# enoche/MMRec

Hardware: AMD Instinct MI355X
Metric: GCN-layer edges/sec (3-layer user-item CSR SpMM, d=64, fp32) (higher is better)
Workload: dtype f32

## Files before the change

include/mmrec_hip.h:

```cpp
#ifndef MMREC_HIP_H
#define MMREC_HIP_H

#include <stddef.h>
#include <stdint.h>

#ifdef __cplusplus
extern "C" {
#endif

#define MMREC_ABI_VERSION 16
#define MMREC_EMB_DIM 64

#define MMREC_ERR_BAD_ARG 10001
#define MMREC_ERR_UNSUPPORTED 10002

typedef void* mmrec_stream_t;

int mmrec_abi_version(void);
const char* mmrec_error_string(int err);

#ifndef MMREC_SPMM_CHUNK
#define MMREC_SPMM_CHUNK 512
#endif
#define MMREC_SPMM_LONG_ROW_DEFAULT 32

int mmrec_spmm_csr_f32(const int32_t* rowptr, const int32_t* colidx, const float* vals,
                       const float* X, float* Y, const float* Z, const float* acc_in, float* acc_out,
                       int32_t n_rows, int32_t d, float alpha, float beta, float acc_scale,
                       int32_t long_row_threshold, const int32_t* long_rows,
                       const int32_t* long_chunk_ptr, int32_t n_long, int32_t n_chunks,
                       float* partials, int32_t* long_tickets, mmrec_stream_t stream);

int mmrec_spmm_rows_f32(const int32_t* rowptr, const int32_t* colidx, const float* vals, const float* X,
                        const float* Z, int32_t z_compact, const int64_t* rows, int32_t n_list, int32_t d,
                        int32_t long_row_threshold, float* Y, mmrec_stream_t stream);
int mmrec_spmm_rows_any_f32(const int32_t* rowptr, const int32_t* colidx, const float* vals, const float* X,
                            const float* Z, int32_t z_compact, const int64_t* rows, int32_t n_list, int32_t d,
                            int32_t long_row_threshold, int32_t max_row_chunks, float* Y, mmrec_stream_t stream);
int mmrec_spmm_push_rows_f32(const int32_t* rowptr, const int32_t* colidx, const float* vals, const float* G,
                             float g_scale, const int64_t* rows, int32_t n_list, int32_t d, float* dX, float* dZ,
                             mmrec_stream_t stream);

int mmrec_spmm_csr_f32_layergcn(const int32_t* rowptr, const int32_t* colidx, const float* vals, const float* X,
                                float* Y, const float* ego, float* scaled, float* w, const float* acc_in,
                                float* acc_out, int32_t n_rows, int32_t d, int32_t long_row_threshold,
                                const int32_t* long_rows, const int32_t* long_chunk_ptr, int32_t n_long,
                                int32_t n_chunks, float* partials, int32_t* long_tickets, mmrec_stream_t stream);
int mmrec_spmm_csr_sched_f32(const int32_t* rowptr, const int32_t* colidx, const float* vals, const float* X, float* Y,
                             const float* Z, const float* acc_in, float* acc_out, int32_t n_rows, int32_t d, float alpha,
                             float beta, float acc_scale, int32_t long_row_threshold, const int32_t* long_rows,
                             const int32_t* long_chunk_ptr, int32_t n_long, int32_t n_chunks, float* partials,
                             int32_t* long_tickets, const int32_t* sched_row, const int32_t* sched_span,
                             const int32_t* sched_col, const float* sched_val, int32_t n_short, mmrec_stream_t stream);
int mmrec_spmm_csr_sched_f32_layergcn(const int32_t* rowptr, const int32_t* colidx, const float* vals, const float* X,
                                      float* Y, const float* ego, float* scaled, float* w, const float* acc_in,
                                      float* acc_out, int32_t n_rows, int32_t d, int32_t long_row_threshold,
                                      const int32_t* long_rows, const int32_t* long_chunk_ptr, int32_t n_long,
                                      int32_t n_chunks, float* partials, int32_t* long_tickets, const int32_t* sched_row,
                                      const int32_t* sched_span, const int32_t* sched_col, const float* sched_val,
                                      int32_t n_short, mmrec_stream_t stream);
int mmrec_spmm_row_keys(const int32_t* rowptr, const int32_t* colidx, const int32_t* col_degree, int32_t n_rows,
                        int32_t long_row_threshold, int32_t key_deg_max, int32_t* key, int32_t* key_degree,
                        mmrec_stream_t stream);

int mmrec_spmm_csr_masked_f32(const int32_t* rowptr, const int32_t* colidx, const float* vals, const float* X, float* Y,
                              const float* Z, const float* acc_in, float* acc_out, int32_t n_rows, int32_t d, float alpha,
                              float beta, float acc_scale, int32_t long_row_threshold, const int32_t* long_rows,
                              const int32_t* long_chunk_ptr, int32_t n_long, int32_t n_chunks, float* partials,
                              int32_t* long_tickets, const uint32_t* keep_bits, float val_scale, mmrec_stream_t stream);
int mmrec_edge_keep_bits(const uint8_t* keep, int64_t n_edges, const int64_t* perm_a, uint32_t* bits_a,
                         const int64_t* perm_b, uint32_t* bits_b, mmrec_stream_t stream);
int mmrec_spmm_plan_count(const int32_t* rowptr_host, int32_t n_rows, int32_t long_row_threshold,
                          int32_t* n_long, int32_t* n_chunks);
int mmrec_spmm_plan_fill(const int32_t* rowptr_host, int32_t n_rows, int32_t long_row_threshold,
                         int32_t* long_rows, int32_t* long_chunk_ptr);

int mmrec_cos_scale_fwd_f32(const float* E, const float* Ego, float* Out, float* w, float* acc,
                            int32_t n_rows, int32_t d, mmrec_stream_t stream);
int mmrec_cos_scale_bwd_f32(const float* dOut, const float* E, const float* Ego, const float* w,
                            float* dE, float* dEgo_accum, int32_t n_rows, int32_t d,
                            mmrec_stream_t stream);

#define MMREC_BPR_LOGSIG 0
#define MMREC_BPR_GAMMA 1

size_t mmrec_bpr_workspace_bytes(int32_t batch);
int mmrec_bpr_fwd_f32(const float* U, const float* P, const float* N, const int64_t* users,
                      const int64_t* pos, const int64_t* neg, int32_t batch, int32_t d,
                      int32_t variant, float scale, float* loss_out, float* coef, void* workspace,
                      mmrec_stream_t stream);
int mmrec_bpr_bwd_f32(const float* U, const float* P, const float* N, const int64_t* users,
                      const int64_t* pos, const int64_t* neg, int32_t batch, int32_t d,
                      const float* coef, const float* grad_scalar, float scale, float* dU, float* dP,
                      float* dN, mmrec_stream_t stream);

int mmrec_bpr_dots_f32(const float* U, const float* P, const float* N, const int64_t* users,
                       const int64_t* pos, const int64_t* neg, int32_t batch, int32_t d, float* dots,
                       mmrec_stream_t stream);
int mmrec_bpr_loss_from_dots_f32(const float* dots, int32_t batch, int32_t variant, float scale,
                                 float* loss_out, float* coef, void* workspace, mmrec_stream_t stream);

int mmrec_gather_sqnorm_fwd_f32(const float* E, const int64_t* ids, int32_t batch, int32_t d,
                                float* out, void* workspace, mmrec_stream_t stream);
int mmrec_gather_scale_add_bwd_f32(const float* E, const int64_t* ids, int32_t batch, int32_t d,
                                   const float* coef_scalar, float* dE, mmrec_stream_t stream);
#define MMREC_ROWS_REG_MAX_TERMS 6
size_t mmrec_rows_reg_workspace_bytes(int32_t n_terms, int32_t max_batch);
int mmrec_rows_reg_fwd_f32(const float* const* E, const int64_t* const* ids, const int32_t* batch, int32_t n_terms, int32_t d,
                           int32_t mode, float scale, float* out, float* coef, void* workspace, mmrec_stream_t stream);
int mmrec_rows_reg_bwd_f32(const float* const* E, const int64_t* const* ids, const int32_t* batch, int32_t n_terms, int32_t d,
                           const float* coef, const float* g, float* const* dE, mmrec_stream_t stream);

#define MMREC_BPR_MAX_TERMS 4
size_t mmrec_bpr_multi_workspace_bytes(int32_t n_terms, int32_t batch);
int mmrec_bpr_multi_fwd_f32(const float* U, const int64_t* users, const float* const* I, const int64_t* const* pos,
                            const int64_t* const* neg, const float* w, int32_t n_terms, int32_t batch, int32_t d, int32_t variant,
                            float scale, float* total, float* losses, float* coef, void* workspace, mmrec_stream_t stream);
int mmrec_bpr_multi_bwd_f32(const float* U, const int64_t* users, const float* const* I, const int64_t* const* pos,
                            const int64_t* const* neg, const float* w, int32_t n_terms, int32_t batch, int32_t d, const float* coef,
                            const float* grad_scalar, float scale, float* dU, float* const* dI, mmrec_stream_t stream);

#define MMREC_COSINE_MAX_TERMS 8
size_t mmrec_cosine_multi_workspace_bytes(int32_t n_terms, int32_t max_batch);
int mmrec_cosine_multi_fwd_f32(const float* const* X, const int64_t* const* ix, const float* const* Y, const int64_t* const* iy,
                               const float* w, const int32_t* batch, int32_t n_terms, int32_t d, float* out, float* coef,
                               void* workspace, mmrec_stream_t stream);
int mmrec_cosine_multi_bwd_f32(const float* const* X, const int64_t* const* ix, const float* const* Y, const int64_t* const* iy,
                               const float* w, const int32_t* batch, int32_t n_terms, int32_t d, const float* coef,
// ... 229 lines not shown
```

mmrec_amd/_lib.py:

```python
from __future__ import annotations

import ctypes
import os
from ctypes import c_char_p, c_float, c_int32, c_int64, c_size_t, c_uint64, c_void_p

import torch

_PKG = os.path.dirname(os.path.abspath(__file__))
LIB_PATH = os.environ.get("MMREC_HIP_LIB") or os.path.join(_PKG, "lib", "libmmrec_hip.so")
ABI_VERSION = 16

_P = c_void_p

SIGNATURES = {
    "mmrec_abi_version": (c_int32, []),
    "mmrec_error_string": (c_char_p, [c_int32]),
    "mmrec_spmm_csr_f32": (c_int32, [_P, _P, _P, _P, _P, _P, _P, _P, c_int32, c_int32, c_float,
                                     c_float, c_float, c_int32, _P, _P, c_int32, c_int32, _P, _P, _P]),
    "mmrec_spmm_csr_f32_layergcn": (c_int32, [_P, _P, _P, _P, _P, _P, _P, _P, _P, _P, c_int32, c_int32, c_int32,
                                              _P, _P, c_int32, c_int32, _P, _P, _P]),
    "mmrec_spmm_csr_sched_f32": (c_int32, [_P, _P, _P, _P, _P, _P, _P, _P, c_int32, c_int32, c_float,
                                           c_float, c_float, c_int32, _P, _P, c_int32, c_int32, _P, _P,
                                           _P, _P, _P, _P, c_int32, _P]),
    "mmrec_spmm_csr_sched_f32_layergcn": (c_int32, [_P, _P, _P, _P, _P, _P, _P, _P, _P, _P, c_int32, c_int32, c_int32,
                                                    _P, _P, c_int32, c_int32, _P, _P, _P, _P, _P, _P, c_int32, _P]),
    "mmrec_spmm_csr_masked_f32": (c_int32, [_P, _P, _P, _P, _P, _P, _P, _P, c_int32, c_int32, c_float,
                                            c_float, c_float, c_int32, _P, _P, c_int32, c_int32, _P, _P, _P, c_float, _P]),
    "mmrec_edge_keep_bits": (c_int32, [_P, c_int64, _P, _P, _P, _P, _P]),
    "mmrec_spmm_row_keys": (c_int32, [_P, _P, _P, c_int32, c_int32, c_int32, _P, _P, _P]),
    "mmrec_spmm_plan_count": (c_int32, [_P, c_int32, c_int32, _P, _P]),
    "mmrec_spmm_plan_fill": (c_int32, [_P, c_int32, c_int32, _P, _P]),
    "mmrec_cos_scale_fwd_f32": (c_int32, [_P, _P, _P, _P, _P, c_int32, c_int32, _P]),
    "mmrec_cos_scale_bwd_f32": (c_int32, [_P, _P, _P, _P, _P, _P, c_int32, c_int32, _P]),
    "mmrec_bpr_workspace_bytes": (c_size_t, [c_int32]),
    "mmrec_bpr_fwd_f32": (c_int32, [_P, _P, _P, _P, _P, _P, c_int32, c_int32, c_int32, c_float, _P,
                                    _P, _P, _P]),
    "mmrec_spmm_rows_f32": (c_int32, [_P, _P, _P, _P, _P, c_int32, _P, c_int32, c_int32, c_int32, _P, _P]),
    "mmrec_spmm_rows_any_f32": (c_int32, [_P, _P, _P, _P, _P, c_int32, _P, c_int32, c_int32, c_int32, c_int32, _P, _P]),
    "mmrec_spmm_push_rows_f32": (c_int32, [_P, _P, _P, _P, c_float, _P, c_int32, c_int32, _P, _P, _P]),
    "mmrec_bpr_dots_f32": (c_int32, [_P, _P, _P, _P, _P, _P, c_int32, c_int32, _P, _P]),
    "mmrec_bpr_loss_from_dots_f32": (c_int32, [_P, c_int32, c_int32, c_float, _P, _P, _P, _P]),
    "mmrec_bpr_bwd_f32": (c_int32, [_P, _P, _P, _P, _P, _P, c_int32, c_int32, _P, _P, c_float, _P, _P,
                                    _P, _P]),
    "mmrec_gather_sqnorm_fwd_f32": (c_int32, [_P, _P, c_int32, c_int32, _P, _P, _P]),
    "mmrec_gather_scale_add_bwd_f32": (c_int32, [_P, _P, c_int32, c_int32, _P, _P, _P]),
    "mmrec_infonce_workspace_bytes": (c_size_t, [c_int32]),
    "mmrec_infonce_fwd_f32": (c_int32, [_P, _P, _P, c_int32, c_int32, c_float, _P, _P, _P]),
    "mmrec_infonce_bwd_f32": (c_int32, [_P, c_int32, c_int32, c_float, _P, _P, _P, _P, _P]),
    "mmrec_linear_workspace_bytes": (c_size_t, [c_int32, c_int32, c_int32]),
    "mmrec_linear_fwd_f32": (c_int32, [_P, _P, _P, _P, c_int32, c_int32, c_int32, _P, _P]),
    "mmrec_linear_fwd_split_f32": (c_int32, [_P, _P, _P, _P, c_int32, c_int32, c_int32, _P, _P]),
    "mmrec_linear_bwd_split_workspace_bytes": (c_size_t, [c_int32, c_int32, c_int32]),
    "mmrec_linear_bwd_split_f32": (c_int32, [_P, _P, _P, _P, _P, _P, c_int32, c_int32, c_int32, _P, _P]),
    "mmrec_linear_bwd_w_f32": (c_int32, [_P, _P, _P, _P, c_int32, c_int32, c_int32, _P, _P]),
    "mmrec_linear_bwd_x_f32": (c_int32, [_P, _P, _P, c_int32, c_int32, c_int32, _P]),
    "mmrec_linear_rows_workspace_bytes": (c_size_t, [c_int32, c_int32, c_int32]),
    "mmrec_linear_rows_fwd_f32": (c_int32, [_P, c_int64, _P, _P, _P, _P, c_int32, c_int32, c_int32, c_int32, _P, _P]),
    "mmrec_linear_rows_bwd_f32": (c_int32, [_P, _P, c_int64, _P, _P, _P, _P, _P, c_int32, c_int32, c_int32, _P, _P]),
    "mmrec_edge_dot_f32": (c_int32, [_P, c_int64, _P, c_int64, _P, _P, c_int64, c_int32, _P, _P]),
    "mmrec_edge_dot_bwd_f32": (c_int32, [_P, _P, c_int64, _P, c_int64, _P, _P, c_int64, c_int32, _P, _P, _P]),
    "mmrec_segment_softmax_group_max": (c_int32, []),
    "mmrec_segment_softmax_f32": (c_int32, [_P, c_int32, _P, _P, c_int32, _P, c_int64, c_float, _P, _P]),
    "mmrec_segment_softmax_bwd_f32": (c_int32, [_P, c_int32, _P, _P, c_int32, _P, _P, c_int64, _P, _P]),
    "mmrec_edge_attention_group_max": (c_int32, []),
    "mmrec_edge_attention_f32": (c_int32, [_P, c_int32, _P, _P, _P, c_int32, _P, c_int64, _P, c_int64, c_int32, c_int64, c_float,
                                           _P, _P, _P]),
    "mmrec_edge_attention_bwd_f32": (c_int32, [_P, c_int32, _P, _P, _P, c_int32, _P, _P, _P, _P, c_int32, _P, c_int64, _P, c_int64,
                                               _P, _P, _P, _P, c_int32, c_int64, _P, _P, _P, _P, _P]),
    "mmrec_neighbor_max_group_max": (c_int32, []),
    "mmrec_neighbor_max_f32": (c_int32, [_P, c_int32, _P, _P, _P, c_int32, _P, c_int64, c_int32, c_int64, _P, _P, _P]),
    "mmrec_neighbor_max_bwd_f32": (c_int32, [_P, c_int32, _P, _P, _P, c_int32, _P, c_int64, _P, c_int32, c_int64, _P, _P, _P]),
    "mmrec_score_lse_split_cols": (c_int32, [c_int32, c_int32, c_int32]),
    "mmrec_score_lse_workspace_bytes": (c_size_t, [c_int32, c_int32, c_int32]),
    "mmrec_score_lse_f32": (c_int32, [_P, _P, c_int32, c_int32, c_int32, c_float, _P, _P, _P]),
    "mmrec_score_lse_bwd_f32": (c_int32, [_P, _P, c_int32, c_int32, c_int32, c_float, _P, _P, _P, _P, _P, _P]),
    "mmrec_hyper_rows_per_block": (c_int32, [c_int64]),
    "mmrec_hyper_workspace_bytes": (c_size_t, [c_int64, c_int64, c_int32]),
    "mmrec_hyper_assign_fwd_f32": (c_int32, [_P, _P, _P, c_int64, c_int32, c_float, c_float, _P, _P, _P]),
    "mmrec_hyper_assign_bwd_f32": (c_int32, [_P, _P, _P, c_int64, c_int32, c_float, c_float, _P, _P]),
    "mmrec_hyper_layer_fwd_f32": (c_int32, [_P, _P, _P, c_int64, c_int64, c_int32, c_int32, _P, _P, _P, _P, _P]),
    "mmrec_hyper_layer_bwd_f32": (c_int32, [_P, _P, _P, _P, _P, _P, c_int64, c_int64, c_int32, c_int32, _P, _P, _P, _P, _P]),
    "mmrec_spectrum_rows_per_block": (c_int32, [c_int64]),
    "mmrec_spectrum_workspace_bytes": (c_size_t, [c_int64]),
    "mmrec_spectrum_fwd_f32": (c_int32, [_P, _P, _P, _P, _P, c_int64, c_int32, _P, _P, _P, _P]),
# ... 102 lines not shown
```

mmrec_amd/csrc/spmm.hip:

```cpp
#include "common.h"
#include "spmm_narrow.h"

#ifndef MMREC_SPMM_RPG
#define MMREC_SPMM_RPG(n_rows) ((n_rows) <= (1 << 18) ? 1 : 4)
#endif

namespace {

__device__ __forceinline__ void st_coherent(float4* p, float4 v) {
    unsigned long long* q = reinterpret_cast<unsigned long long*>(p);
    const unsigned long long lo = ((unsigned long long)__float_as_uint(v.y) << 32) | __float_as_uint(v.x);
    const unsigned long long hi = ((unsigned long long)__float_as_uint(v.w) << 32) | __float_as_uint(v.z);
    __hip_atomic_store(q, lo, __ATOMIC_RELAXED, __HIP_MEMORY_SCOPE_AGENT);
    __hip_atomic_store(q + 1, hi, __ATOMIC_RELAXED, __HIP_MEMORY_SCOPE_AGENT);
}
__device__ __forceinline__ float4 ld_coherent(const float4* p) {
    unsigned long long* q = reinterpret_cast<unsigned long long*>(const_cast<float4*>(p));
    const unsigned long long lo = __hip_atomic_load(q, __ATOMIC_RELAXED, __HIP_MEMORY_SCOPE_AGENT);
    const unsigned long long hi = __hip_atomic_load(q + 1, __ATOMIC_RELAXED, __HIP_MEMORY_SCOPE_AGENT);
    return make_float4(__uint_as_float((unsigned)lo), __uint_as_float((unsigned)(lo >> 32)),
                       __uint_as_float((unsigned)hi), __uint_as_float((unsigned)(hi >> 32)));
}

struct RowEpilogue {
// ... 151 lines not shown
            } else {
#pragma unroll
                for (int ch = 0; ch < DCH; ++ch) {
                    float4* dst = reinterpret_cast<float4*>(partials) + (size_t)chunk * (16 * DCH) + ch * 16 + lane16;
                    if (tickets) st_coherent(dst, t[ch]); else *dst = t[ch];
                }
            }
        }
        const int c0 = long_chunk_ptr[lo], c1 = long_chunk_ptr[lo + 1];
        if (!tickets || c1 - c0 == 1) return;
        if (threadIdx.x < 64) {
            __atomic_signal_fence(__ATOMIC_SEQ_CST);
            __builtin_amdgcn_s_waitcnt(0);
            __atomic_signal_fence(__ATOMIC_SEQ_CST);
            __builtin_amdgcn_fence(__ATOMIC_RELEASE, "workgroup");
            if (threadIdx.x == 0)
                s_last = __hip_atomic_fetch_add(tickets + lo, 1, __ATOMIC_RELAXED, __HIP_MEMORY_SCOPE_AGENT) == c1 - c0 - 1;
        }
        __syncthreads();
        if (!s_last) return;
        __builtin_amdgcn_fence(__ATOMIC_ACQUIRE, "workgroup");
        reduce_long_row<DCH, true, LG>(partials, c0, c1, row, ep, red);
        if (threadIdx.x == 0) __hip_atomic_store(tickets + lo, 0, __ATOMIC_RELAXED, __HIP_MEMORY_SCOPE_AGENT);
        return;
    }
    if (SCHED) {
        const int slot0 = ((int)blockIdx.x - n_chunks) * 16 * rows_per_group + g;
#pragma unroll 1
        for (int i = 0; i < rows_per_group; ++i) {
            const int slot = slot0 + i * 16;
            if (slot >= sched.n_short) break;
            const int row = sched.row[slot];
            const int2 se = sched.span[slot];
            float4 acc[DCH];
#pragma unroll
            for (int ch = 0; ch < DCH; ++ch) acc[ch] = f4_zero();
            gather_span<DCH>(sched.col, sched.val, X4, se.x, se.y, lane16, acc);
            store_row<DCH, LG>(ep, row, lane16, acc);
        }
        return;
    }
    const int row0 = ((int)blockIdx.x - n_chunks) * 16 * rows_per_group + g;
#pragma unroll 1
    for (int i = 0; i < rows_per_group; ++i) {
        const int row = row0 + i * 16;
        if (row >= n_rows) break;
        const int s = rowptr[row], e = rowptr[row + 1];
        if (e - s > long_t) continue;
        float4 acc[DCH];
#pragma unroll
        for (int ch = 0; ch < DCH; ++ch) acc[ch] = f4_zero();
        gather_span<DCH>(colidx, vals, X4, s, e, lane16, acc);
        store_row<DCH, LG>(ep, row, lane16, acc);
    }
}

template <int DCH, bool LG>
__global__ __launch_bounds__(256) void spmm_long_reduce_kernel(
    const int32_t* __restrict__ long_rows, const int32_t* __restrict__ long_chunk_ptr, int n_long,
    const float* __restrict__ partials, RowEpilogue ep) {
    __shared__ float4 red[16][16 * DCH];
    const int i = blockIdx.x;
    const int c0 = long_chunk_ptr[i], c1 = long_chunk_ptr[i + 1];
    if (c1 - c0 <= 1) return;
    reduce_long_row<DCH, false, LG>(partials, c0, c1, long_rows[i], ep, red);
}

template <int DCH, bool LG = false, bool SCHED = false>
void launch_spmm(hipStream_t s, int blocks, int nch, const int32_t* rowptr, const int32_t* colidx,
                 const float* vals, const float* X, const RowEpilogue& ep, int n_rows, int long_t,
                 int rows_per_group, const int32_t* long_rows, const int32_t* long_chunk_ptr, int n_long,
                 float* partials, int32_t* tickets, const RowSchedule& sched = RowSchedule{}) {
    if (blocks + nch > 0)
        hipLaunchKernelGGL((spmm_rows_kernel<DCH, LG, SCHED>), dim3(blocks + nch), dim3(256), 0, s, rowptr, colidx, vals, X,
                           ep, n_rows, long_t, rows_per_group, long_rows, long_chunk_ptr, n_long, nch, partials, tickets,
                           sched);
    if (!tickets && n_long > 0 && nch > n_long)
        hipLaunchKernelGGL((spmm_long_reduce_kernel<DCH, LG>), dim3(n_long), dim3(256), 0, s, long_rows,
                           long_chunk_ptr, n_long, partials, ep);
}

template <int DCH>
__device__ __forceinline__ void gather_span_masked(const int32_t* __restrict__ colidx, const float* __restrict__ vals,
                                                   const uint32_t* __restrict__ keep_bits, float val_scale,
                                                   const float4* __restrict__ X4, int s, int e, int lane16,
                                                   float4 (&acc)[DCH]) {
    constexpr int NB = DCH == 1 ? 8 : (DCH <= 2 ? 4 : (DCH <= 4 ? 2 : 1));
    const int gshift = threadIdx.x & 48;
    for (int base = s; base < e; base += 16) {
        const int k = base + lane16;
        int c = 0;
        float v = 0.f;
        bool kept = false;
        if (k < e) {
            kept = (keep_bits[k >> 5] >> (k & 31)) & 1u;
            c = colidx[k];
            v = vals[k] * val_scale;
        }
        unsigned m = (unsigned)(__ballot(kept) >> gshift) & 0xffffu;
        while (m) {
            float4 x[NB][DCH];
            float vv[NB];
#pragma unroll
            for (int u = 0; u < NB; ++u) {
                const bool on = m != 0;
                const int j = on ? __ffs(m) - 1 : 0;
// ... 381 lines not shown
    if (n_long > 0 && (!long_rows || !long_chunk_ptr || !partials || n_chunks <= 0))
        return MMREC_ERR_BAD_ARG;
    if (!sched_args_ok(sched_row, sched_span, sched_col, sched_val, n_short, n_rows)) return MMREC_ERR_BAD_ARG;
    if (Y == X || acc_out == X) return MMREC_ERR_BAD_ARG;
    RowEpilogue ep{Z, Y, acc_in, acc_out, alpha, Z ? beta : 0.f, acc_scale, nullptr, nullptr, nullptr};
    const RowSchedule sched{sched_row, reinterpret_cast<const int2*>(sched_span), sched_col, sched_val, n_short};
    hipStream_t s = mmrec_stream(stream);
    const int rows_per_group = MMREC_SPMM_RPG(n_rows);
    const int blocks = (n_short + 16 * rows_per_group - 1) / (16 * rows_per_group);
    const int long_t = n_long > 0 ? long_row_threshold : INT32_MAX;
    const int nch = n_long > 0 ? n_chunks : 0;
    int32_t* tickets = n_long > 0 ? long_tickets : nullptr;
#define MMREC_SPMM_CASE(D)                                                                                      \
    case D:                                                                                                     \
        launch_spmm<D, false, true>(s, blocks, nch, rowptr, colidx, vals, X, ep, n_rows, long_t, rows_per_group, \
                                    long_rows, long_chunk_ptr, n_long, partials, tickets, sched);               \
        break;
    switch (d / MMREC_EMB_DIM) {
        MMREC_SPMM_CASE(1) MMREC_SPMM_CASE(2) MMREC_SPMM_CASE(3) MMREC_SPMM_CASE(4) MMREC_SPMM_CASE(5)
        MMREC_SPMM_CASE(6)
    }
#undef MMREC_SPMM_CASE
    MMREC_RETURN_LAUNCH_STATUS();
}

extern "C" int mmrec_spmm_csr_sched_f32_layergcn(const int32_t* rowptr, const int32_t* colidx, const float* vals,
                                                 const float* X, float* Y, const float* ego, float* scaled, float* w,
                                                 const float* acc_in, float* acc_out, int32_t n_rows, int32_t d,
                                                 int32_t long_row_threshold, const int32_t* long_rows,
                                                 const int32_t* long_chunk_ptr, int32_t n_long, int32_t n_chunks,
                                                 float* partials, int32_t* long_tickets, const int32_t* sched_row,
                                                 const int32_t* sched_span, const int32_t* sched_col,
                                                 const float* sched_val, int32_t n_short, mmrec_stream_t stream) {
    if (d != MMREC_EMB_DIM) return MMREC_ERR_UNSUPPORTED;
    if (n_rows < 0 || n_long < 0 || n_chunks < 0 || long_row_threshold < 0) return MMREC_ERR_BAD_ARG;
    if (n_rows == 0) return 0;
    if (!rowptr || !X || !ego || !scaled || !w) return MMREC_ERR_BAD_ARG;
    if (n_long > 0 && (!long_rows || !long_chunk_ptr || !partials || n_chunks <= 0)) return MMREC_ERR_BAD_ARG;
    if (!sched_args_ok(sched_row, sched_span, sched_col, sched_val, n_short, n_rows)) return MMREC_ERR_BAD_ARG;
    if (Y == X || scaled == X || acc_out == X) return MMREC_ERR_BAD_ARG;
    RowEpilogue ep{nullptr, Y, acc_in, acc_out, 1.f, 0.f, 1.f, ego, scaled, w};
    const RowSchedule sched{sched_row, reinterpret_cast<const int2*>(sched_span), sched_col, sched_val, n_short};
    hipStream_t s = mmrec_stream(stream);
    const int rows_per_group = MMREC_SPMM_RPG(n_rows);
    const int blocks = (n_short + 16 * rows_per_group - 1) / (16 * rows_per_group);
    const int long_t = n_long > 0 ? long_row_threshold : INT32_MAX;
    const int nch = n_long > 0 ? n_chunks : 0;
    int32_t* tickets = n_long > 0 ? long_tickets : nullptr;
    launch_spmm<1, true, true>(s, blocks, nch, rowptr, colidx, vals, X, ep, n_rows, long_t, rows_per_group, long_rows,
                               long_chunk_ptr, n_long, partials, tickets, sched);
    MMREC_RETURN_LAUNCH_STATUS();
}

extern "C" int mmrec_spmm_row_keys(const int32_t* rowptr, const int32_t* colidx, const int32_t* col_degree,
                                   int32_t n_rows, int32_t long_row_threshold, int32_t key_deg_max, int32_t* key,
                                   int32_t* key_degree, mmrec_stream_t stream) {
    if (n_rows < 0 || long_row_threshold < 0 || key_deg_max < 0) return MMREC_ERR_BAD_ARG;
    if (n_rows == 0) return 0;
    if (!rowptr || !colidx || !col_degree || !key || !key_degree) return MMREC_ERR_BAD_ARG;
    hipLaunchKernelGGL(spmm_row_keys_kernel, dim3((n_rows + 15) / 16), dim3(256), 0, mmrec_stream(stream), rowptr, colidx,
                       col_degree, n_rows, long_row_threshold, key_deg_max, key, key_degree);
    MMREC_RETURN_LAUNCH_STATUS();
}

extern "C" int mmrec_spmm_plan_count(const int32_t* rowptr_host, int32_t n_rows,
                                     int32_t long_row_threshold, int32_t* n_long, int32_t* n_chunks) {
    if (!rowptr_host || !n_long || !n_chunks || n_rows < 0) return MMREC_ERR_BAD_ARG;
    int32_t nl = 0, nc = 0;
    for (int32_t r = 0; r < n_rows; ++r) {
        const int32_t deg = rowptr_host[r + 1] - rowptr_host[r];
        if (deg > long_row_threshold) {
            ++nl;
            nc += (deg + MMREC_SPMM_CHUNK - 1) / MMREC_SPMM_CHUNK;
        }
    }
    *n_long = nl;
    *n_chunks = nc;
    return 0;
}

extern "C" int mmrec_spmm_plan_fill(const int32_t* rowptr_host, int32_t n_rows,
                                    int32_t long_row_threshold, int32_t* long_rows,
                                    int32_t* long_chunk_ptr) {
    if (!rowptr_host || !long_rows || !long_chunk_ptr || n_rows < 0) return MMREC_ERR_BAD_ARG;
    int32_t nl = 0, nc = 0;
    for (int32_t r = 0; r < n_rows; ++r) {
        const int32_t deg = rowptr_host[r + 1] - rowptr_host[r];
        if (deg > long_row_threshold) {
            long_rows[nl] = r;
            long_chunk_ptr[nl] = nc;
            ++nl;
            nc += (deg + MMREC_SPMM_CHUNK - 1) / MMREC_SPMM_CHUNK;
        }
    }
    long_chunk_ptr[nl] = nc;
    return 0;
}

extern "C" int mmrec_cos_scale_fwd_f32(const float* E, const float* Ego, float* Out, float* w,
                                       float* acc, int32_t n_rows, int32_t d, mmrec_stream_t stream) {
    if (d != MMREC_EMB_DIM) return MMREC_ERR_UNSUPPORTED;
    if (n_rows < 0 || (n_rows > 0 && (!E || !Ego || !Out || !w))) return MMREC_ERR_BAD_ARG;
    if (n_rows == 0) return 0;
    hipLaunchKernelGGL(cos_scale_fwd_kernel, dim3((n_rows + 15) / 16), dim3(256), 0,
                       mmrec_stream(stream), E, Ego, Out, w, acc, n_rows);
    MMREC_RETURN_LAUNCH_STATUS();
}

extern "C" int mmrec_cos_scale_bwd_f32(const float* dOut, const float* E, const float* Ego,
                                       const float* w, float* dE, float* dEgo_accum, int32_t n_rows,
                                       int32_t d, mmrec_stream_t stream) {
    if (d != MMREC_EMB_DIM) return MMREC_ERR_UNSUPPORTED;
    if (n_rows < 0 || (n_rows > 0 && (!dOut || !E || !Ego || !w || !dE || !dEgo_accum)))
        return MMREC_ERR_BAD_ARG;
    if (n_rows == 0) return 0;
    hipLaunchKernelGGL(cos_scale_bwd_kernel, dim3((n_rows + 15) / 16), dim3(256), 0,
                       mmrec_stream(stream), dOut, E, Ego, w, dE, dEgo_accum, n_rows);
    MMREC_RETURN_LAUNCH_STATUS();
}
```

mmrec_amd/hip_ops.py:

```python
from __future__ import annotations

import ctypes
import math

import numpy as np
import torch

from . import _lib

EMB_DIM = 64
LINEAR_F16X3_DEFAULT = True
LINEAR_F16X3 = LINEAR_F16X3_DEFAULT
SLICE_WIDTHS = (8, 16, 32)
SPMM_CHUNK = 512
LONG_ROW_DEFAULT = None


def default_long_row_threshold(n_cols):
    import os
    forced = os.environ.get("MMREC_LONG_ROW_THRESHOLD")
    if forced:
        return int(forced)
    return 16 if n_cols <= (1 << 18) else 32


ROW_SCHEDULE_MIN_COLS = 1 << 18
SPMM_KEY_DEG_MAX = 128


def spmm_key_deg_max():
    import os
    forced = os.environ.get("MMREC_SPMM_KEY_DEG_MAX")
    return int(forced) if forced else SPMM_KEY_DEG_MAX


TOPK_MAX = 128
BPR_LOGSIG, BPR_GAMMA = 0, 1

DETERMINISTIC_DEFAULT = False
DETERMINISTIC = DETERMINISTIC_DEFAULT
_TORCH_DET_BY_US = False


def set_deterministic(flag=True):
    global DETERMINISTIC, _TORCH_DET_BY_US
    DETERMINISTIC = bool(flag)
    if DETERMINISTIC and not torch.are_deterministic_algorithms_enabled():
        torch.use_deterministic_algorithms(True, warn_only=True)
        _TORCH_DET_BY_US = True
    elif not DETERMINISTIC and _TORCH_DET_BY_US:
        torch.use_deterministic_algorithms(False)
        _TORCH_DET_BY_US = False


def scatter_add_rows(ids, rows, out):
    lib = _lib.load()
    _chk(ids, torch.int64, "ids", 1)
    rows, out = _chk(rows.contiguous(), torch.float32, "rows", 2), _chk(out, torch.float32, "out", 2)
    order = torch.sort(ids, stable=True)[1]
    _lib.check(lib.mmrec_scatter_add_rows_sorted_f32(_p(order), _p(ids), _p(rows), ids.numel(), rows.shape[1], _p(out),
                                                     _stream()), "scatter_add_rows_sorted")
    return out


def _p(t):
    return None if t is None else ctypes.c_void_p(t.data_ptr())


def _stream():
    return ctypes.c_void_p(torch.cuda.current_stream().cuda_stream)


def _chk(t, dtype, name, dim=None):
    if not isinstance(t, torch.Tensor) or not t.is_cuda:
        raise _lib.MMRecHipError("%s must be a device tensor (the hot path has no CPU fallback)" % name)
    if t.dtype != dtype:
        raise _lib.MMRecHipError("%s must be %s, got %s" % (name, dtype, t.dtype))
    if not t.is_contiguous():
        raise _lib.MMRecHipError("%s must be contiguous" % name)
    if dim is not None and t.dim() != dim:
        raise _lib.MMRecHipError("%s must be %d-d" % (name, dim))
    return t


def _ws(nbytes, device):
    return torch.empty(max(int(nbytes), 16), dtype=torch.uint8, device=device)
# ... 31 lines not shown
            cp = np.empty(self.n_long + 1, dtype=np.int32)
            _lib.check(lib.mmrec_spmm_plan_fill(rp.ctypes.data_as(ctypes.c_void_p), self.n_rows,
                                                self.long_row_threshold,
                                                lr.ctypes.data_as(ctypes.c_void_p),
                                                cp.ctypes.data_as(ctypes.c_void_p)), "spmm_plan_fill")
            self.long_rows = torch.from_numpy(lr).to(dev)
            self.long_chunk_ptr = torch.from_numpy(cp).to(dev)
            self.max_row_chunks = int(np.diff(cp).max())
            self.long_tickets = torch.zeros(self.n_long, dtype=torch.int32, device=dev)
        else:
            self.long_rows = self.long_chunk_ptr = self.long_tickets = None
            self.max_row_chunks = 1
        self._partials = {}
        self.sched = None
        if self.row_schedule:
            self._plan_schedule()

    def _plan_schedule(self):
        lib = _lib.load()
        dev, n = self.rowptr.device, self.n_rows
        deg = (self.rowptr[1:] - self.rowptr[:-1])
        short = torch.nonzero(deg <= self.long_row_threshold).squeeze(1)
        key = torch.full((n,), -1, dtype=torch.int32, device=dev)
        kdeg = torch.zeros(n, dtype=torch.int32, device=dev)
        if self.nnz > 0 and n > 0:
            if self.symmetric and self.n_cols == n:
                coldeg = deg.contiguous()
            else:
                coldeg = torch.bincount(self.colidx, minlength=self.n_cols).to(torch.int32)
            _lib.check(lib.mmrec_spmm_row_keys(_p(self.rowptr), _p(self.colidx), _p(coldeg), n, self.long_row_threshold,
                                               spmm_key_deg_max(), _p(key), _p(kdeg), _stream()), "spmm_row_keys")
        self.row_key, self.row_key_degree = key, kdeg
        k, kd, dg = key[short].long(), kdeg[short].long(), deg[short].long()
        first = self.colidx[self.rowptr[:-1][short].long().clamp_(max=max(self.nnz - 1, 0))].long() if self.nnz > 0 else k
        ref = torch.where(k >= 0, k, torch.where(dg > 0, first, torch.full_like(k, -1)))
        band = (ref <= short).long()
        comp = (band << 62) | (((1 << 31) - 1 - kd) << 31) | k.clamp(min=0)
        order = torch.sort(comp, stable=True)[1]
        rows = short[order]
        lens = dg[order]
        end = torch.cumsum(lens, 0)
        begin = end - lens
        total = int(end[-1].item()) if rows.numel() else 0
        src0 = self.rowptr[:-1].long()[rows]
        pos = torch.arange(total, dtype=torch.int64, device=dev) + torch.repeat_interleave(src0 - begin, lens, output_size=total)
        self.sched = {
            "row": rows.to(torch.int32).contiguous(),
            "span": torch.stack([begin, end], 1).to(torch.int32).contiguous(),
            "col": self.colidx.index_select(0, pos) if total else torch.zeros(1, dtype=torch.int32, device=dev),
            "val": self.vals.index_select(0, pos) if total else torch.zeros(1, dtype=torch.float32, device=dev),
            "n_short": int(rows.numel()),
            "vals_of": self.vals,
        }

    def scheduled(self, d):
        sc = self.sched
        return sc if sc is not None and d % EMB_DIM == 0 and sc["vals_of"] is self.vals else None

    def schedule_bytes(self):
        return 0 if self.sched is None else sum(self.sched[k].numel() * self.sched[k].element_size() for k in ("row", "span", "col", "val"))

    def checked(self, rc, what):
        try:
            _lib.check(rc, what)
        except _lib.MMRecHipError:
            if self.long_tickets is not None:
                try:
                    self.long_tickets.zero_()
                except RuntimeError:
                    pass
            raise

    def partials_for(self, d):
        if self.n_long == 0:
            return None
        if d not in self._partials:
            self._partials[d] = torch.empty(self.n_chunks * d, dtype=torch.float32, device=self.rowptr.device)
        return self._partials[d]

    @classmethod
    def from_coo_host(cls, idx, val, n_rows, n_cols, device, symmetric=False, **kw):
        idx = np.asarray(idx, dtype=np.int64)
        val = np.asarray(val, dtype=np.float32)
        order = np.argsort(idx[0], kind="stable")
        rowptr = np.zeros(n_rows + 1, dtype=np.int64)
        np.cumsum(np.bincount(idx[0], minlength=n_rows), out=rowptr[1:])
        rp = rowptr.astype(np.int32)
        return cls(torch.from_numpy(rp).to(device),
                   torch.from_numpy(idx[1][order].astype(np.int32)).to(device),
                   torch.from_numpy(val[order]).to(device), n_rows, n_cols, symmetric=symmetric,
                   rowptr_host=rp, **kw)

    @classmethod
    def from_coo_device(cls, rows, cols, vals, n_rows, n_cols, symmetric=False, **kw):
        lib = _lib.load()
        _chk(rows, torch.int32, "rows", 1), _chk(cols, torch.int32, "cols", 1)
        _chk(vals, torch.float32, "vals", 1)
        nnz, dev = rows.numel(), rows.device
        rowptr = torch.empty(n_rows + 1, dtype=torch.int32, device=dev)
        colidx = torch.empty(nnz, dtype=torch.int32, device=dev)
        vout = torch.empty(nnz, dtype=torch.float32, device=dev)
        ws = _ws(lib.mmrec_coo_to_csr_workspace_bytes(nnz, n_rows), dev)
        _lib.check(lib.mmrec_coo_to_csr(_p(rows), _p(cols), _p(vals), nnz, n_rows, _p(rowptr),
                                        _p(colidx), _p(vout), _p(ws), _stream()), "coo_to_csr")
        return cls(rowptr, colidx, vout, n_rows, n_cols, symmetric=symmetric, **kw)

# ... 80 lines not shown
        lab = np.arange(n, dtype=np.int64)
        sides = [slice(None)] if not n_left else [rows < n_left, rows >= n_left]
        for _ in range(int(iters)):
            for side in sides:
                new = _mode_labels(rows[side], lab[ci[side]], n, n)
                lab = np.where(new >= 0, new, lab)
        order = np.lexsort((np.arange(n), lab))
    else:
        raise ValueError("reorder must be 'degree', 'rcm' or 'community', got %r" % (how,))
    perm = np.empty(n, dtype=np.int64)
    perm[order] = np.arange(n, dtype=np.int64)
    return perm


class PermutedGraph:

    def __init__(self, g: CsrGraph, reorder, n_left=None):
        if g.n_rows != g.n_cols:
            raise _lib.MMRecHipError("PermutedGraph needs a square graph")
        dev, n = g.rowptr.device, g.n_rows
        idx, val = g.to_coo_host()
        perm = locality_order(g.rowptr_host, idx[1], n, reorder, n_left=n_left)
        self.base, self.reorder = g, reorder
        self.perm = torch.from_numpy(perm).to(dev)
        inv = np.empty(n, dtype=np.int64)
        inv[perm] = np.arange(n, dtype=np.int64)
        self.inv = torch.from_numpy(inv).to(dev)
        self.graph = CsrGraph.from_coo_host(np.stack([perm[idx[0]], perm[idx[1]]]), val, n, n, dev, symmetric=g.symmetric,
                                            long_row_threshold=g.long_row_threshold)
        self.n_rows = self.n_cols = n
        self.nnz = g.nnz

    def to_new(self, X):
        return X.index_select(0, self.inv)

    def to_old(self, Xp):
        return Xp.index_select(0, self.perm)


def spmm_raw(g: CsrGraph, X, Y=None, Z=None, acc_in=None, acc_out=None, alpha=1.0, beta=1.0,
             acc_scale=1.0):
    lib = _lib.load()
    _chk(X, torch.float32, "X", 2)
    d = X.shape[1]
    if (d not in SLICE_WIDTHS and (d % EMB_DIM or d > 6 * EMB_DIM)) or X.shape[0] < g.n_cols:
        raise _lib.MMRecHipError("X must be [>=%d, 64*k <= 384 (or a feature slice of 8 / 16 / 32 columns)], got %s" %
                                 (g.n_cols, tuple(X.shape)))
    for t, nm in ((Y, "Y"), (Z, "Z"), (acc_in, "acc_in"), (acc_out, "acc_out")):
        if t is not None:
            _chk(t, torch.float32, nm, 2)
            if t.shape[0] < g.n_rows or t.shape[1] != d:
                raise _lib.MMRecHipError("%s must be [>=%d, %d]" % (nm, g.n_rows, d))
    sc = g.scheduled(d)
    if sc is not None:
        g.checked(lib.mmrec_spmm_csr_sched_f32(_p(g.rowptr), _p(g.colidx), _p(g.vals), _p(X), _p(Y), _p(Z),
                                               _p(acc_in), _p(acc_out), g.n_rows, d, float(alpha),
                                               float(beta), float(acc_scale), g.long_row_threshold,
                                               _p(g.long_rows), _p(g.long_chunk_ptr), g.n_long, g.n_chunks,
                                               _p(g.partials_for(d)), _p(g.long_tickets), _p(sc["row"]), _p(sc["span"]),
                                               _p(sc["col"]), _p(sc["val"]), sc["n_short"], _stream()), "spmm_csr_sched_f32")
        return Y if Y is not None else acc_out
    g.checked(lib.mmrec_spmm_csr_f32(_p(g.rowptr), _p(g.colidx), _p(g.vals), _p(X), _p(Y), _p(Z),
                                     _p(acc_in), _p(acc_out), g.n_rows, d, float(alpha),
                                     float(beta), float(acc_scale), g.long_row_threshold,
                                     _p(g.long_rows), _p(g.long_chunk_ptr), g.n_long, g.n_chunks,
                                     _p(g.partials_for(d)), _p(g.long_tickets), _stream()), "spmm_csr_f32")
    return Y if Y is not None else acc_out


ROWS_MAX_CHUNKS = 480


def rows_servable(g: CsrGraph, d):
    if d not in SLICE_WIDTHS + (EMB_DIM,):
        return False
    return g.n_chunks == g.n_long or (d == EMB_DIM and g.max_row_chunks <= ROWS_MAX_CHUNKS)


def spmm_rows_raw(g: CsrGraph, X, rows, Z=None, z_compact=False):
    lib = _lib.load()
    _chk(X, torch.float32, "X", 2), _chk(rows, torch.int64, "rows", 1)
    d = X.shape[1]
    if not rows_servable(g, d) or X.shape[0] < g.n_cols:
        raise _lib.MMRecHipError("spmm_rows: graph with multi-chunk rows, or X not [>=%d, 8 / 16 / 32 / 64]" % g.n_cols)
    if Z is not None and (_chk(Z, torch.float32, "Z", 2).shape[0] < (rows.numel() if z_compact else g.n_rows) or Z.shape[1] != d):
        raise _lib.MMRecHipError("Z must be [>=%d, %d]" % (rows.numel() if z_compact else g.n_rows, d))
    Y = torch.empty(rows.numel(), d, dtype=torch.float32, device=X.device)
    long_t = g.long_row_threshold if g.n_long > 0 else 2 ** 31 - 1
    if g.n_chunks == g.n_long:
        _lib.check(lib.mmrec_spmm_rows_f32(_p(g.rowptr), _p(g.colidx), _p(g.vals), _p(X), _p(Z), 1 if z_compact else 0, _p(rows),
                                           rows.numel(), d, long_t, _p(Y), _stream()), "spmm_rows_f32")
    else:
        _lib.check(lib.mmrec_spmm_rows_any_f32(_p(g.rowptr), _p(g.colidx), _p(g.vals), _p(X), _p(Z), 1 if z_compact else 0, _p(rows),
                                               rows.numel(), d, long_t, g.max_row_chunks, _p(Y), _stream()), "spmm_rows_any_f32")
    return Y


def spmm_push_rows_raw(g: CsrGraph, G, rows, dX=None, dZ=None, scale=1.0):
    lib = _lib.load()
    _chk(G, torch.float32, "G", 2), _chk(rows, torch.int64, "rows", 1)
    d = G.shape[1]
    if G.shape[0] != rows.numel() or d not in SLICE_WIDTHS + (EMB_DIM,):
        raise _lib.MMRecHipError("G must be [len(rows), 8 / 16 / 32 / 64]")
    for t, nm, n in ((dX, "dX", g.n_cols), (dZ, "dZ", g.n_rows)):
        if t is not None and (_chk(t, torch.float32, nm, 2).shape[0] < n or t.shape[1] != d):
            raise _lib.MMRecHipError("%s must be [>=%d, %d]" % (nm, n, d))
# ... 2248 lines not shown
```

Before: 31.23 billion.

## Add precomputed work-item descriptors for a unified SpMM launch

Builds a host-side list of per-block work items, either chunks of long rows or groups of up to 16/64 short scheduled rows. A single new items kernel then processes both kinds in one launch, using a prefix-end array instead of begin/end spans. The goal is to remove per-block scheduling arithmetic and to balance long-row chunks alongside short-row blocks. In exchange it adds host planning at graph setup and an extra descriptor read per block. It also adds a workgroup-wide reduction path for long rows.

```diff
diff --git a/include/mmrec_hip.h b/include/mmrec_hip.h
--- a/include/mmrec_hip.h
+++ b/include/mmrec_hip.h
@@ -74,6 +74,17 @@
                           int32_t* n_long, int32_t* n_chunks);
 int mmrec_spmm_plan_fill(const int32_t* rowptr_host, int32_t n_rows, int32_t long_row_threshold,
                          int32_t* long_rows, int32_t* long_chunk_ptr);
+#define MMREC_SPMM_ITEM_INTS 8
+#define MMREC_SPMM_ITEM_CHUNK 0
+#define MMREC_SPMM_ITEM_ROWS 1
+int mmrec_spmm_desc_build(const int32_t* rowptr_host, int32_t n_rows, int32_t long_row_threshold,
+                          const int32_t* sched_row, const int32_t* sched_key, int32_t n_short, int32_t block_rows,
+                          int32_t tail_blocks, int32_t* items, int32_t* sched_end, int32_t* n_items);
+int mmrec_spmm_csr_items_f32(const int32_t* colidx, const float* vals, const float* X, float* Y, const float* Z,
+                             const float* acc_in, float* acc_out, int32_t n_rows, int32_t d, float alpha, float beta,
+                             float acc_scale, const int32_t* items, int32_t n_items, int32_t n_chunks, float* partials,
+                             int32_t* long_tickets, const int32_t* sched_row, const int32_t* sched_end,
+                             const int32_t* sched_col, const float* sched_val, int32_t n_short, mmrec_stream_t stream);
 
 int mmrec_cos_scale_fwd_f32(const float* E, const float* Ego, float* Out, float* w, float* acc,
                             int32_t n_rows, int32_t d, mmrec_stream_t stream);
diff --git a/mmrec_amd/_lib.py b/mmrec_amd/_lib.py
--- a/mmrec_amd/_lib.py
+++ b/mmrec_amd/_lib.py
@@ -30,6 +30,9 @@
     "mmrec_spmm_row_keys": (c_int32, [_P, _P, _P, c_int32, c_int32, c_int32, _P, _P, _P]),
     "mmrec_spmm_plan_count": (c_int32, [_P, c_int32, c_int32, _P, _P]),
     "mmrec_spmm_plan_fill": (c_int32, [_P, c_int32, c_int32, _P, _P]),
+    "mmrec_spmm_desc_build": (c_int32, [_P, c_int32, c_int32, _P, _P, c_int32, c_int32, c_int32, _P, _P, _P]),
+    "mmrec_spmm_csr_items_f32": (c_int32, [_P, _P, _P, _P, _P, _P, _P, c_int32, c_int32, c_float, c_float, c_float,
+                                           _P, c_int32, c_int32, _P, _P, _P, _P, _P, _P, c_int32, _P]),
     "mmrec_cos_scale_fwd_f32": (c_int32, [_P, _P, _P, _P, _P, c_int32, c_int32, _P]),
     "mmrec_cos_scale_bwd_f32": (c_int32, [_P, _P, _P, _P, _P, _P, c_int32, c_int32, _P]),
     "mmrec_bpr_workspace_bytes": (c_size_t, [c_int32]),
diff --git a/mmrec_amd/csrc/spmm.hip b/mmrec_amd/csrc/spmm.hip
--- a/mmrec_amd/csrc/spmm.hip
+++ b/mmrec_amd/csrc/spmm.hip
@@ -227,6 +227,85 @@
         for (int ch = 0; ch < DCH; ++ch) acc[ch] = f4_zero();
         gather_span<DCH>(colidx, vals, X4, s, e, lane16, acc);
         store_row<DCH, LG>(ep, row, lane16, acc);
+    }
+}
+
+struct SpmmItem {
+    int32_t kind;
+    int32_t a, b, c, d, e, f, g;
+};
+static_assert(sizeof(SpmmItem) == 4 * MMREC_SPMM_ITEM_INTS, "one item is MMREC_SPMM_ITEM_INTS int32");
+
+#ifndef MMREC_SPMM_ITEMS_WAVES
+#define MMREC_SPMM_ITEMS_WAVES 7
+#endif
+template <int DCH>
+__global__ __launch_bounds__(256) __attribute__((amdgpu_waves_per_eu(1, MMREC_SPMM_ITEMS_WAVES))) void spmm_items_kernel(
+    const SpmmItem* __restrict__ items, const int32_t* __restrict__ colidx, const float* __restrict__ vals,
+    const float* __restrict__ X, RowEpilogue ep, float* __restrict__ partials, int32_t* __restrict__ tickets,
+    const int32_t* __restrict__ sched_row, const int32_t* __restrict__ sched_end, const int32_t* __restrict__ sched_col,
+    const float* __restrict__ sched_val) {
+    __shared__ float4 red[16][16 * DCH];
+    __shared__ int s_last;
+    const int lane16 = threadIdx.x & 15;
+    const int g = threadIdx.x >> 4;
+    const float4* X4 = reinterpret_cast<const float4*>(X);
+    const SpmmItem it = items[blockIdx.x];
+    if (it.kind == MMREC_SPMM_ITEM_CHUNK) {
+        const int row = it.a, cs = it.b, ce = it.c, lo = it.d, c0 = it.e, c1 = it.f, chunk = it.g;
+        float4 acc[DCH];
+#pragma unroll
+        for (int ch = 0; ch < DCH; ++ch) acc[ch] = f4_zero();
+        for (int base = cs + g * 16; base < ce; base += 256)
+            gather_span<DCH>(colidx, vals, X4, base, min(base + 16, ce), lane16, acc);
+#pragma unroll
+        for (int ch = 0; ch < DCH; ++ch) red[g][ch * 16 + lane16] = acc[ch];
+        __syncthreads();
+        if (g == 0) {
+            float4 t[DCH];
+#pragma unroll
+            for (int ch = 0; ch < DCH; ++ch) {
+                t[ch] = red[0][ch * 16 + lane16];
+#pragma unroll
+                for (int i = 1; i < 16; ++i) t[ch] = f4_add(t[ch], red[i][ch * 16 + lane16]);
+            }
+            if (c1 - c0 == 1) {
+                store_row<DCH, false>(ep, row, lane16, t);
+            } else {
+#pragma unroll
+                for (int ch = 0; ch < DCH; ++ch) {
+                    float4* dst = reinterpret_cast<float4*>(partials) + (size_t)chunk * (16 * DCH) + ch * 16 + lane16;
+                    st_coherent(dst, t[ch]);
+                }
+            }
+        }
+        if (c1 - c0 == 1) return;
+        if (threadIdx.x < 64) {
+            __atomic_signal_fence(__ATOMIC_SEQ_CST);
+            __builtin_amdgcn_s_waitcnt(0);
+            __atomic_signal_fence(__ATOMIC_SEQ_CST);
+            __builtin_amdgcn_fence(__ATOMIC_RELEASE, "workgroup");
+            if (threadIdx.x == 0)
+                s_last = __hip_atomic_fetch_add(tickets + lo, 1, __ATOMIC_RELAXED, __HIP_MEMORY_SCOPE_AGENT) == c1 - c0 - 1;
+        }
+        __syncthreads();
+        if (!s_last) return;
+        __builtin_amdgcn_fence(__ATOMIC_ACQUIRE, "workgroup");
+        reduce_long_row<DCH, true, false>(partials, c0, c1, row, ep, red);
+        if (threadIdx.x == 0) __hip_atomic_store(tickets + lo, 0, __ATOMIC_RELAXED, __HIP_MEMORY_SCOPE_AGENT);
+        return;
+    }
+    const int first = it.a, count = it.b;
+#pragma unroll 1
+    for (int i = g; i < count; i += 16) {
+        const int slot = first + i;
+        const int row = sched_row[slot];
+        const int s = slot > 0 ? sched_end[slot - 1] : 0, e = sched_end[slot];
+        float4 acc[DCH];
+#pragma unroll
+        for (int ch = 0; ch < DCH; ++ch) acc[ch] = f4_zero();
+        gather_span<DCH>(sched_col, sched_val, X4, s, e, lane16, acc);
+        store_row<DCH, false>(ep, row, lane16, acc);
     }
 }
 
@@ -714,6 +793,37 @@
     MMREC_RETURN_LAUNCH_STATUS();
 }
 
+extern "C" int mmrec_spmm_csr_items_f32(const int32_t* colidx, const float* vals, const float* X, float* Y, const float* Z,
+                                        const float* acc_in, float* acc_out, int32_t n_rows, int32_t d, float alpha,
+                                        float beta, float acc_scale, const int32_t* items, int32_t n_items,
+                                        int32_t n_chunks, float* partials, int32_t* long_tickets,
+                                        const int32_t* sched_row, const int32_t* sched_end, const int32_t* sched_col,
+                                        const float* sched_val, int32_t n_short, mmrec_stream_t stream) {
+    if (d <= 0 || d % MMREC_EMB_DIM || d / MMREC_EMB_DIM > 6) return MMREC_ERR_UNSUPPORTED;
+    if (n_rows < 0 || n_items < 0 || n_chunks < 0 || n_chunks > n_items) return MMREC_ERR_BAD_ARG;
+    if (n_rows == 0) return 0;
+    if (!X || (!Y && !acc_out) || !items || n_items == 0) return MMREC_ERR_BAD_ARG;
+    if (acc_out && !acc_in) return MMREC_ERR_BAD_ARG;
+    if (n_chunks > 0 && (!colidx || !vals || !partials || !long_tickets)) return MMREC_ERR_BAD_ARG;
+    if (n_short < 0 || n_short > n_rows || (n_short == 0) != (n_items == n_chunks)) return MMREC_ERR_BAD_ARG;
+    if (n_short > 0 && (!sched_row || !sched_end || !sched_col || !sched_val)) return MMREC_ERR_BAD_ARG;
+    if (Y == X || acc_out == X) return MMREC_ERR_BAD_ARG;
+    RowEpilogue ep{Z, Y, acc_in, acc_out, alpha, Z ? beta : 0.f, acc_scale, nullptr, nullptr, nullptr};
+    hipStream_t s = mmrec_stream(stream);
+#define MMREC_SPMM_CASE(D)                                                                                               \
+    case D:                                                                                                              \
+        hipLaunchKernelGGL((spmm_items_kernel<D>), dim3(n_items), dim3(256), 0, s,                                       \
+                           reinterpret_cast<const SpmmItem*>(items), colidx, vals, X, ep, partials, long_tickets, sched_row, \
+                           sched_end, sched_col, sched_val);                                                             \
+        break;
+    switch (d / MMREC_EMB_DIM) {
+        MMREC_SPMM_CASE(1) MMREC_SPMM_CASE(2) MMREC_SPMM_CASE(3) MMREC_SPMM_CASE(4) MMREC_SPMM_CASE(5)
+        MMREC_SPMM_CASE(6)
+    }
+#undef MMREC_SPMM_CASE
+    MMREC_RETURN_LAUNCH_STATUS();
+}
+
 extern "C" int mmrec_spmm_row_keys(const int32_t* rowptr, const int32_t* colidx, const int32_t* col_degree,
                                    int32_t n_rows, int32_t long_row_threshold, int32_t key_deg_max, int32_t* key,
                                    int32_t* key_degree, mmrec_stream_t stream) {
@@ -759,6 +869,73 @@
     return 0;
 }
 
+extern "C" int mmrec_spmm_desc_build(const int32_t* rowptr_host, int32_t n_rows, int32_t long_row_threshold,
+                                     const int32_t* sched_row, const int32_t* sched_key, int32_t n_short,
+                                     int32_t block_rows, int32_t tail_blocks, int32_t* items, int32_t* sched_end,
+                                     int32_t* n_items) {
+    if (!rowptr_host || !n_items || n_rows < 0 || long_row_threshold < 0) return MMREC_ERR_BAD_ARG;
+    if (n_short < 0 || n_short > n_rows || (n_short > 0 && !sched_row)) return MMREC_ERR_BAD_ARG;
+    if (block_rows < 16 || block_rows > 64 || block_rows % 16 || tail_blocks < 0) return MMREC_ERR_BAD_ARG;
+    int64_t n = 0;
+    auto put = [&](int32_t kind, int32_t a, int32_t b, int32_t c, int32_t d, int32_t e, int32_t f, int32_t g) {
+        if (items && n < INT32_MAX) {
+            const int32_t v[MMREC_SPMM_ITEM_INTS] = {kind, a, b, c, d, e, f, g};
+            for (int i = 0; i < MMREC_SPMM_ITEM_INTS; ++i) items[n * MMREC_SPMM_ITEM_INTS + i] = v[i];
+        }
+        ++n;
+    };
+    int32_t nl = 0, nc = 0;
+    for (int32_t r = 0; r < n_rows; ++r) {
+        const int32_t deg = rowptr_host[r + 1] - rowptr_host[r];
+        if (deg <= long_row_threshold) continue;
+        const int32_t k = (deg + MMREC_SPMM_CHUNK - 1) / MMREC_SPMM_CHUNK;
+        for (int32_t c = 0; c < k; ++c) {
+            const int32_t cs = rowptr_host[r] + c * MMREC_SPMM_CHUNK;
+            put(MMREC_SPMM_ITEM_CHUNK, r, cs, c + 1 < k ? cs + MMREC_SPMM_CHUNK : rowptr_host[r + 1], nl, nc, nc + k, nc + c);
+        }
+        ++nl;
+        nc += k;
+    }
+    int64_t end = 0;
+    for (int32_t s = 0; s < n_short; ++s) {
+        const int32_t r = sched_row[s];
+        if (r < 0 || r >= n_rows) return MMREC_ERR_BAD_ARG;
+        const int32_t deg = rowptr_host[r + 1] - rowptr_host[r];
+        if (deg < 0 || deg > long_row_threshold) return MMREC_ERR_BAD_ARG;
+        end += deg;
+        if (end > INT32_MAX) return MMREC_ERR_BAD_ARG;
+        if (sched_end) sched_end[s] = (int32_t)end;
+    }
+    const int64_t tail_start = (int64_t)n_short - 16 * (int64_t)tail_blocks;
+    const auto cap_at = [&](int32_t s) { return s >= tail_start ? 16 : block_rows; };
+    int32_t first = 0, fill = 0, cap = 0;
+    for (int32_t s = 0; s < n_short;) {
+        int32_t e = s + 1;
+        if (sched_key && sched_key[s] >= 0) {
+            const bool band = sched_key[s] <= sched_row[s];
+            while (e < n_short && sched_key[e] == sched_key[s] && (sched_key[e] <= sched_row[e]) == band) ++e;
+        }
+        if (fill > 0 && e - s > cap - fill && e - s <= cap_at(s)) {
+            put(MMREC_SPMM_ITEM_ROWS, first, fill, 0, 0, 0, 0, 0);
+            fill = 0;
+        }
+        while (s < e) {
+            if (fill == 0) first = s, cap = cap_at(s);
+            const int32_t take = e - s < cap - fill ? e - s : cap - fill;
+            fill += take;
+            s += take;
+            if (fill == cap) {
+                put(MMREC_SPMM_ITEM_ROWS, first, fill, 0, 0, 0, 0, 0);
+                fill = 0;
+            }
+        }
+    }
+    if (fill > 0) put(MMREC_SPMM_ITEM_ROWS, first, fill, 0, 0, 0, 0, 0);
+    if (n > INT32_MAX) return MMREC_ERR_BAD_ARG;
+    *n_items = (int32_t)n;
+    return 0;
+}
+
 extern "C" int mmrec_cos_scale_fwd_f32(const float* E, const float* Ego, float* Out, float* w,
                                        float* acc, int32_t n_rows, int32_t d, mmrec_stream_t stream) {
     if (d != MMREC_EMB_DIM) return MMREC_ERR_UNSUPPORTED;
diff --git a/mmrec_amd/hip_ops.py b/mmrec_amd/hip_ops.py
--- a/mmrec_amd/hip_ops.py
+++ b/mmrec_amd/hip_ops.py
@@ -32,6 +32,16 @@
     import os
     forced = os.environ.get("MMREC_SPMM_KEY_DEG_MAX")
     return int(forced) if forced else SPMM_KEY_DEG_MAX
+
+
+SPMM_ITEMS = True
+SPMM_ITEM_INTS = 8
+
+
+def spmm_items_on():
+    import os
+    forced = os.environ.get("MMREC_SPMM_ITEMS")
+    return forced != "0" if forced else SPMM_ITEMS
 
 
 TOPK_MAX = 128
@@ -169,6 +179,26 @@
             "n_short": int(rows.numel()),
             "vals_of": self.vals,
         }
+        self.plan_items()
+
+    def plan_items(self, block_rows=None, tail_blocks=0, group_cuts=False):
+        lib, sc, dev = _lib.load(), self.sched, self.rowptr.device
+        if block_rows is None:
+            block_rows = 16 if self.n_rows <= (1 << 18) else 64
+        rows = np.ascontiguousarray(sc["row"].cpu().numpy())
+        keys = np.ascontiguousarray(self.row_key[sc["row"].long()].cpu().numpy()) if group_cuts else None
+        hp = lambda a: None if a is None else a.ctypes.data_as(ctypes.c_void_p)
+        n_items = ctypes.c_int32(0)
+
+        def build(items, end):
+            _lib.check(lib.mmrec_spmm_desc_build(hp(self.rowptr_host), self.n_rows, self.long_row_threshold, hp(rows), hp(keys),
+                                                 sc["n_short"], block_rows, tail_blocks, hp(items), hp(end),
+                                                 ctypes.byref(n_items)), "spmm_desc_build")
+        build(None, None)
+        items = np.empty((n_items.value, SPMM_ITEM_INTS), dtype=np.int32)
+        end = np.empty(max(sc["n_short"], 1), dtype=np.int32)
+        build(items, end)
+        sc["items"], sc["end"], sc["n_items"] = torch.from_numpy(items).to(dev), torch.from_numpy(end).to(dev), n_items.value
 
     def scheduled(self, d):
         sc = self.sched
@@ -355,6 +385,13 @@
             if t.shape[0] < g.n_rows or t.shape[1] != d:
                 raise _lib.MMRecHipError("%s must be [>=%d, %d]" % (nm, g.n_rows, d))
     sc = g.scheduled(d)
+    if sc is not None and spmm_items_on() and (g.n_long == 0 or g.long_tickets is not None):
+        g.checked(lib.mmrec_spmm_csr_items_f32(_p(g.colidx), _p(g.vals), _p(X), _p(Y), _p(Z), _p(acc_in), _p(acc_out), g.n_rows,
+                                               d, float(alpha), float(beta), float(acc_scale), _p(sc["items"]), sc["n_items"],
+                                               g.n_chunks, _p(g.partials_for(d)), _p(g.long_tickets), _p(sc["row"]),
+                                               _p(sc["end"]), _p(sc["col"]), _p(sc["val"]), sc["n_short"], _stream()),
+                  "spmm_csr_items_f32")
+        return Y if Y is not None else acc_out
     if sc is not None:
         g.checked(lib.mmrec_spmm_csr_sched_f32(_p(g.rowptr), _p(g.colidx), _p(g.vals), _p(X), _p(Y), _p(Z),
                                                _p(acc_in), _p(acc_out), g.n_rows, d, float(alpha),
```

Result: no change. 31.48 billion, median of 6 (+0.8%).
